# hangg7/soar

Measured on AMD Instinct MI355X. Metric: fwd+bwd frames/sec @100k Gaussians, 1080p; achieved HBM GB/s vs roofline, higher is better.
Workload: dtype f32

## Files before the change

include/soar_hip.h:

```cpp
#ifndef SOAR_HIP_H
#define SOAR_HIP_H

#include <stddef.h>
#include <stdint.h>

#ifdef __cplusplus
extern "C" {
#endif

#define SOAR_HIP_ABI_VERSION 8

typedef struct SoarRastParams {
    int32_t P;
    int32_t W, H;
    int32_t sh_degree;
    int32_t M;
    int32_t prefiltered;
    int32_t render_front;
    int32_t sort_descending;
    int32_t debug;
    int32_t cfg_surface;
    int32_t cfg_normalize_depth;
    int32_t cfg_perpix_depth;
    int32_t cfg_lrn_cam;
// ... 202 lines not shown
} SoarLossFinish;
int soar_frames_geometry_warp_backward_losses(int32_t n, const SoarFrameTail *frames, const float *xyz, const float *rot,
                                              const float *weights, const float *joint_mats, int32_t P, int32_t J, const float *scales,
                                              float *dL_dxyz, float *dL_drot, float *dL_dscales, float *dL_dcolors, float *dL_docc,
                                              const SoarLossFinish *finish, void *stream);

int soar_lbs_warp_forward_batch(const float *xyz, const float *rot, const float *weights, const float *joint_mats, int32_t n,
                                int32_t P, int32_t J, float *xyz_out, float *rot_out, void *stream);
int soar_lbs_warp_backward_sum(const float *xyz, const float *rot, const float *weights, const float *joint_mats, int32_t n,
                               int32_t P, int32_t J, const float *dL_dxyz_out, const float *dL_drot_out, float *dL_dxyz,
                               float *dL_drot, int32_t n_extra, const float *const *extra_src, float *const *extra_dst,
                               const int32_t *extra_width, void *stream);

int soar_dist2_knn3(const float *points, int32_t N, float *out, void *stream);

#define SOAR_FRAME_LOSS_SCRATCH_FLOATS (4 * 2048)
int soar_frame_loss(int32_t W, int32_t H, const float *color, const float *normal, const float *depth,
                    const float *opac, const float *target_color, const float *target_mask,
                    const float *target_normal, float w_color, float w_mask, float w_normal, float w_depth,
                    float *loss_out, float *scratch, float *dL_dcolor, float *dL_dnormal, float *dL_ddepth,
                    float *dL_dopac, const void *image_buffer, const float *background, int32_t normalize_depth, void *stream);

int soar_frame_loss_pooled(int32_t W, int32_t H, const float *color, const float *normal, const float *depth,
                           const float *opac, const float *target_pool, int32_t n_sets, const int32_t *set_index_dev,
                           float w_color, float w_mask, float w_normal, float w_depth, float *loss_out, float *scratch,
                           float *dL_dcolor, float *dL_dnormal, float *dL_ddepth, float *dL_dopac, const void *image_buffer,
                           const float *background, int32_t normalize_depth, void *stream);
int soar_frame_loss_partials(int32_t W, int32_t H, const float *color, const float *normal, const float *depth,
                             const float *opac, const float *target_color, const float *target_mask,
                             const float *target_normal, float w_color, float w_mask, float w_normal, float w_depth,
// ... 854 lines not shown
```

soar_amd/csrc/geom_bwd_point.h:

```cpp
#pragma once
#include "soar_common.h"
#include "soar_m3.h"

namespace soar {

namespace {

__constant__ float bSH_C0 = 0.28209479177387814f;
__constant__ float bSH_C1 = 0.4886025119029199f;
__constant__ float bSH_C2[5] = {1.0925484305920792f, -1.0925484305920792f, 0.31539156525252005f, -1.0925484305920792f,
                                0.5462742152960396f};
__constant__ float bSH_C3[7] = {-0.5900435899266435f, 2.890611442640554f, -0.4570457994644658f, 0.3731763325901154f,
                                -0.4570457994644658f, 1.445305721320277f, -0.5900435899266435f};

struct GeomBwdArgs {
    int P, D, M, W, H;
    int surface, lrn_cam;
    float tanfovx, tanfovy, h_x, h_y, scale_modifier;
    const float *means3D, *shs, *scales, *rotations, *cov3D;
    const int32_t *radii;
    const uint8_t *clamped;
    const float *view, *proj, *campos;
    const float *acc;
    float *dL_dmeans2D, *dL_dcolors, *dL_dopacity, *dL_dmeans3D, *dL_dcov3D, *dL_dsh, *dL_dscales, *dL_drots;
// ... 31 lines not shown
        acc[0] = r0.x; acc[1] = r0.y; acc[2] = r0.z; acc[3] = r0.w;
        acc[4] = r1.x; acc[5] = r1.y; acc[6] = r1.z; acc[7] = r1.w;
        acc[8] = r2.x; acc[9] = r2.y; acc[10] = r2.z; acc[11] = r2.w;
        acc[12] = r3.x; acc[13] = r3.y;
    }
#pragma unroll
    for (int k = 0; k < 3; k++) { g_mean[k] = 0.f; g_scale[k] = 0.f; }
#pragma unroll
    for (int k = 0; k < 6; k++) g_cov[k] = 0.f;
#pragma unroll
    for (int k = 0; k < 4; k++) g_rot[k] = 0.f;
    if (active) {
        const float *V = a.view, *PM = a.proj;
        const float mx = a.means3D[3 * idx], my = a.means3D[3 * idx + 1], mz = a.means3D[3 * idx + 2];

        const float *cov3D = a.cov3D + 6 * idx;
        const float dcon0 = acc[2], dcon1 = acc[3], dcon2 = acc[4];
        float t0 = V[0] * mx + V[4] * my + V[8] * mz + V[12];
        float t1 = V[1] * mx + V[5] * my + V[9] * mz + V[13];
        float t2 = V[2] * mx + V[6] * my + V[10] * mz + V[14];
        const float limx = 1.3f * a.tanfovx, limy = 1.3f * a.tanfovy;
        const float txtz = t0 / t2, tytz = t1 / t2;
        t0 = fminf(limx, fmaxf(-limx, txtz)) * t2;
        t1 = fminf(limy, fmaxf(-limy, tytz)) * t2;
        const float x_grad_mul = (txtz < -limx || txtz > limx) ? 0.f : 1.f;
        const float y_grad_mul = (tytz < -limy || tytz > limy) ? 0.f : 1.f;
        const float J0 = a.h_x / t2, J1 = -(a.h_x * t0) / (t2 * t2), J2 = a.h_y / t2, J3 = -(a.h_y * t1) / (t2 * t2);
        M3 Jm, Wm, Vrk;
        Jm.e[0][0] = J0; Jm.e[0][1] = 0.f; Jm.e[0][2] = J1;
        Jm.e[1][0] = 0.f; Jm.e[1][1] = J2; Jm.e[1][2] = J3;
        Jm.e[2][0] = 0.f; Jm.e[2][1] = 0.f; Jm.e[2][2] = 0.f;
// ... 123 lines not shown
                }
                ddir[0] += ddx * g; ddir[1] += ddy * g; ddir[2] += ddz * g;
            }
            const float sum2 = ox * ox + oy * oy + oz * oz;
            const float inv32 = 1.0f / sqrtf(sum2 * sum2 * sum2);
            const float gx_ = ((sum2 - ox * ox) * ddir[0] - oy * ox * ddir[1] - oz * ox * ddir[2]) * inv32;
            const float gy_ = (-ox * oy * ddir[0] + (sum2 - oy * oy) * ddir[1] - oz * oy * ddir[2]) * inv32;
            const float gz_ = (-ox * oz * ddir[0] - oy * oz * ddir[1] + (sum2 - oz * oz) * ddir[2]) * inv32;
            g_mean[0] += gx_; g_mean[1] += gy_; g_mean[2] += gz_;
            if ((CAM_SH && a.lrn_cam)) { cam_pos[0] -= gx_; cam_pos[1] -= gy_; cam_pos[2] -= gz_; }
        }

        if (a.scales) {
            const float4 q = reinterpret_cast<const float4 *>(a.rotations)[idx];
            const float r = q.x, x = q.y, y = q.z, z = q.w;
            M3 R, S;
            R.e[0][0] = 1.f - 2.f * (y * y + z * z); R.e[0][1] = 2.f * (x * y - r * z); R.e[0][2] = 2.f * (x * z + r * y);
            R.e[1][0] = 2.f * (x * y + r * z); R.e[1][1] = 1.f - 2.f * (x * x + z * z); R.e[1][2] = 2.f * (y * z - r * x);
            R.e[2][0] = 2.f * (x * z - r * y); R.e[2][1] = 2.f * (y * z + r * x); R.e[2][2] = 1.f - 2.f * (x * x + y * y);
            const float s0 = a.scale_modifier * a.scales[3 * idx], s1 = a.scale_modifier * a.scales[3 * idx + 1],
                        s2 = a.scale_modifier * a.scales[3 * idx + 2];
#pragma unroll
            for (int c = 0; c < 3; c++)
#pragma unroll
                for (int k = 0; k < 3; k++) S.e[c][k] = 0.f;
            S.e[0][0] = s0; S.e[1][1] = s1; S.e[2][2] = s2;
            M3 Mm = m3mul(S, R);
            M3 dSig;
            dSig.e[0][0] = g_cov[0]; dSig.e[0][1] = 0.5f * g_cov[1]; dSig.e[0][2] = 0.5f * g_cov[2];
            dSig.e[1][0] = 0.5f * g_cov[1]; dSig.e[1][1] = g_cov[3]; dSig.e[1][2] = 0.5f * g_cov[4];
            dSig.e[2][0] = 0.5f * g_cov[2]; dSig.e[2][1] = 0.5f * g_cov[4]; dSig.e[2][2] = g_cov[5];
#pragma unroll
            for (int c = 0; c < 3; c++)
#pragma unroll
// ... 29 lines not shown
        }
    }

}

inline void fill_geom_bwd_args(GeomBwdArgs &a, const SoarRastParams &prm, const float *means3D, const int32_t *radii, const float *shs,
                               const float *scales, const float *rotations, const float *cov3D_precomp, const GeomBuf &g, const float *acc)
{
    a.P = prm.P; a.D = prm.sh_degree; a.M = prm.M; a.W = prm.W; a.H = prm.H;
    a.surface = prm.cfg_surface; a.lrn_cam = prm.cfg_lrn_cam;
    a.tanfovx = prm.tanfovx; a.tanfovy = prm.tanfovy;
    a.h_y = prm.H / (2.0f * prm.tanfovy);
    a.h_x = prm.W / (2.0f * prm.tanfovx);
    a.scale_modifier = prm.scale_modifier;
    a.means3D = means3D; a.shs = shs; a.scales = scales; a.rotations = rotations;
    a.cov3D = cov3D_precomp ? cov3D_precomp : g.cov3D;
    a.radii = radii; a.clamped = g.clamped;
    a.view = prm.viewmatrix_dev; a.proj = prm.projmatrix_dev; a.campos = prm.campos_dev;
    a.acc = acc;
}

}

}
```

soar_amd/csrc/lbs.hip:

```cpp
#include "soar_common.h"
#include "loss_finish.h"
#include "geom_bwd_point.h"
#include "preprocess_point.h"
#include "soar_quat.h"

#pragma clang fp contract(on)

#ifndef SOAR_LBS_SKIP_UNUSED_JOINTS
#define SOAR_LBS_SKIP_UNUSED_JOINTS 1
#endif

namespace soar {

namespace {

constexpr int KNN_TILE = 1024;

__device__ __forceinline__ void quat_to_mat(const float q[4], float m[9])
{
    const float r = q[0], i = q[1], j = q[2], k = q[3];
    const float two_s = 2.0f / (r * r + i * i + j * j + k * k);
    m[0] = 1 - two_s * (j * j + k * k); m[1] = two_s * (i * j - k * r); m[2] = two_s * (i * k + j * r);
    m[3] = two_s * (i * j + k * r); m[4] = 1 - two_s * (i * i + k * k); m[5] = two_s * (j * k - i * r);
    m[6] = two_s * (i * k - j * r); m[7] = two_s * (j * k + i * r); m[8] = 1 - two_s * (i * i + j * j);
// ... 346 lines not shown
#pragma unroll
                for (int f = 0; f < WARP_NF; f++) v[c][f] = (c0 + c < w && f < n) ? src[(size_t)f * count + c0 + c] : 0.f;
#pragma unroll
            for (int c = 0; c < 4; c++) {
                if (c0 + c >= w) break;
                float s = v[c][0];
#pragma unroll
                for (int f = 1; f < WARP_NF; f++) s = f < n ? s + v[c][f] : s;
                for (int f = WARP_NF; f < n; f++) s += src[(size_t)f * count + c0 + c];
                dst[c0 + c] = s;
            }
        }
    }
}

__global__ void __launch_bounds__(WARP_THREADS) warp_preprocess_frames_kernel(WarpArgs a, int n, Batch<PreArgs> fr)
{
    extern __shared__ float wtile[];
    const int tid = threadIdx.x, k = __builtin_amdgcn_readfirstlane(tid / WAVE), lane = tid % WAVE;
    const int p0 = blockIdx.x * WAVE, p_raw = p0 + lane;
    stage_weight_rows(a, wtile, tid, p0);
    const int f = blockIdx.y * WARP_NF + k;
    if (f >= n) return;
    const bool in_range = p_raw < a.P;
    const int p = in_range ? p_raw : a.P - 1;
    float M[12], pos[3];
    float4 quat;
    blend_frame_matrix(wtile + (p - p0) * a.J, a.joint_mats + (size_t)f * a.mats_stride, a.J, M);
    forward_point_vals(a, p, M, pos, quat);
    float *xyz_out = a.xyz_out + (size_t)f * a.xyz_stride, *rot_out = a.rot_out + (size_t)f * a.rot_stride;
    xyz_out[3 * p] = pos[0]; xyz_out[3 * p + 1] = pos[1]; xyz_out[3 * p + 2] = pos[2];
    reinterpret_cast<float4 *>(rot_out)[p] = quat;
    const PreArgs &g = fr.v[f];
    PrePoint o;
    preprocess_point(g, p, in_range, pos[0], pos[1], pos[2], true, quat, o);
    preprocess_store(g, p, in_range, blockIdx.x, o);
    if (!g.prefiltered && blockIdx.x == 0 && lane == 0) g.header[H_PREFILTER_VIOLATIONS] = 0u;
}

constexpr int TAIL_C = 14;
struct TailOut {
    float *dL_dmeans2D[MAX_BATCH];
    float *dL_dscales, *dL_dcolors, *dL_docc;
};
struct TailLosses {
    int n, first_block;
    int per_wave;
    SoarLossFinish v[MAX_BATCH];
};
#ifndef SOAR_TAIL_WPE
#define SOAR_TAIL_WPE 4
// ... 47 lines not shown
#pragma unroll
                for (int kk = 0; kk < WARP_NF; kk++) acc[h] += red[kk * TAIL_C * WAVE + o];
        }
    }
#pragma unroll
    for (int h = 0; h < PER; h++) {
        const int o = tid + h * WARP_THREADS, c = o / WAVE, q = p0 + o % WAVE;
        if (o < TAIL_C * WAVE && q < a.P) {
            if (c < 3) a.g_xyz[3 * q + c] = acc[h];
            else if (c < 7) a.g_rot[4 * q + c - 3] = acc[h];
            else if (c < 10) out.dL_dscales[3 * q + c - 7] = acc[h];
            else if (c < 13) out.dL_dcolors[3 * q + c - 10] = acc[h];
            else if (out.dL_docc) out.dL_docc[q] = acc[h];
        }
    }
}

__global__ void __launch_bounds__(256) dist2_knn3_kernel(const float *__restrict__ pts, int N, float *__restrict__ out)
{
    __shared__ float tile[KNN_TILE * 3];
    const int tid = threadIdx.x;
    const int p = blockIdx.x * 256 + tid;
    const bool valid = p < N;
    float x = 0.f, y = 0.f, z = 0.f;
    if (valid) { x = pts[3 * p]; y = pts[3 * p + 1]; z = pts[3 * p + 2]; }
    float b0 = 3.402823466e+38f, b1 = b0, b2 = b0;
    for (int base = 0; base < N; base += KNN_TILE) {
        const int n = min(KNN_TILE, N - base);
        __syncthreads();
        for (int t = tid; t < n * 3; t += 256) tile[t] = pts[(size_t)base * 3 + t];
// ... 153 lines not shown
    a.P = P; a.J = J; a.xyz = xyz; a.rot = rot; a.weights = weights; a.joint_mats = joint_mats;
    a.xyz_out = xyz_out; a.rot_out = rot_out;
    a.mats_stride = (size_t)J * 16; a.xyz_stride = (size_t)P * 3; a.rot_stride = (size_t)P * 4;
    Batch<PreArgs> fr{};
    for (int f = 0; f < n; f++) {
        const SoarFrameHead &t = frames[f];
        if (!t.prm || !t.geom_buffer || !t.radii) { set_error("%s: frame %d: a pointer is NULL", who, f); return 1; }
        if (t.prm->P != P || t.prm->M != 0 || t.prm->prefiltered != 0) {
            set_error("%s: frame %d: needs P = %d Gaussians with explicit colours (M = 0), not prefiltered", who, f, P);
            return 1;
        }
        GeomBuf g;
        carve_geom(t.geom_buffer, P, 0, &g);
        fill_pre_args(fr.v[f], *t.prm, xyz_out + (size_t)f * a.xyz_stride, nullptr, colors, opacities, scales, rot_out + (size_t)f * a.rot_stride,
                      nullptr, g, t.radii);
    }
    const size_t lds = sizeof(float) * WAVE * (size_t)J;
    StageTimer timer(ST_LBS_WARP_FWD, stream);
    hipLaunchKernelGGL(warp_preprocess_frames_kernel, dim3((P + WAVE - 1) / WAVE, (n + WARP_NF - 1) / WARP_NF), dim3(WARP_THREADS), lds, stream,
                       a, (int)n, fr);
    SOAR_LAUNCH_OK("frames_warp_preprocess", stream, 0);
    return 0;
}

int soar_frames_geometry_warp_backward(int32_t n, const SoarFrameTail *frames, const float *xyz, const float *rot, const float *weights,
                                       const float *joint_mats, int32_t P, int32_t J, const float *scales, float *dL_dxyz, float *dL_drot,
                                       float *dL_dscales, float *dL_dcolors, float *dL_docc, void *stream_)
{
    return soar_frames_geometry_warp_backward_losses(n, frames, xyz, rot, weights, joint_mats, P, J, scales, dL_dxyz, dL_drot, dL_dscales,
                                                     dL_dcolors, dL_docc, nullptr, stream_);
}

// ... 61 lines not shown
            if (!l.sums4 || !l.loss_out || l.blocks < 1 || l.blocks > SOAR_FRAME_LOSS_SCRATCH_FLOATS / 4 || l.n < 1) {
                set_error("%s: frame %d: finish[] is not what %s left", who, f,
                          per_wave ? "soar_rast_backward_plan_loss" : "soar_frame_loss_partials");
                return 1;
            }
            losses.v[f] = l;
        }
    }
    const size_t lds = sizeof(float) * (WAVE * (size_t)J + WARP_NF * TAIL_C * WAVE);
    StageTimer timer(ST_LBS_WARP_BWD, stream);
    hipLaunchKernelGGL(geom_warp_backward_frames_kernel, dim3(blocks + losses.n), dim3(WARP_THREADS), lds, stream, a, (int)n, fr, out, losses);
    SOAR_LAUNCH_OK("frames_geometry_warp_backward", stream, 0);
    return 0;
}

int soar_dist2_knn3(const float *points, int32_t N, float *out, void *stream_)
{
    hipStream_t stream = static_cast<hipStream_t>(stream_);
    if (N < 0) { set_error("soar_dist2_knn3: N < 0"); return 1; }
    if (N == 0) return 0;
    if (!points || !out) { set_error("soar_dist2_knn3: NULL pointer"); return 1; }
    StageTimer timer(ST_DIST2, stream);
    hipLaunchKernelGGL(dist2_knn3_kernel, dim3((N + 255) / 256), dim3(256), 0, stream, points, N, out);
    SOAR_LAUNCH_OK("dist2_knn3", stream, 0);
    return 0;
}

}
```

soar_amd/csrc/preprocess_point.h:

```cpp
#pragma once
#include "soar_common.h"
#include "soar_m3.h"

namespace soar {

namespace {

__device__ __forceinline__ float pix_from_ndc(float v, int S, float prcp)
{
#pragma clang fp contract(off)
    return (float)(((v + 1.0) * S - 1.0) * 0.5 + S * (prcp - 0.5));
}

__device__ __forceinline__ float unit3(float *v)
{
#pragma clang fp contract(off)
    float mod = fmaxf(sqrtf(v[0] * v[0] + v[1] * v[1] + v[2] * v[2]), (float)0.00000001);
    v[0] /= mod;
    v[1] /= mod;
    v[2] /= mod;
    return mod;
}

__constant__ float kSH_C0 = 0.28209479177387814f;
// ... 59 lines not shown
    uint8_t *clamped;
    float *front_out;
    uint2 *rect_out;
    uint32_t *depth_key_out;
    uint32_t *blk_stats;
    int32_t *radii;
    uint32_t *header;
};

struct PrePoint {
    GaussRec rec;
    uint2 rect;
    uint32_t depth_key, tiles, key_bits;
    int radius;
    bool alive, faces_camera, prefilter_violation;
};

__device__ __forceinline__ void preprocess_point(const PreArgs &a, const int idx, const bool in_range, const float px3, const float py3,
                                                 const float pz3, const bool has_rot, const float4 q, PrePoint &o)
{
#pragma clang fp contract(off)
    int out_radius = 0;
    uint32_t out_tiles = 0;
    uint2 out_rect = make_uint2(0u, 0u);
    GaussRec rec;
    rec.q0 = make_float4(0.f, 0.f, 0.f, 0.f);
    rec.q1 = rec.q0;
    rec.q2 = rec.q0;
    rec.q3 = rec.q0;

// ... 14 lines not shown
    bool alive = true;
    {
        float x0 = a.bbox[1], y0 = a.bbox[0], x1 = a.bbox[3], y1 = a.bbox[2];
        float w = x1 - x0, h = y1 - y0;
        float expand = (float)0.2;
        if (vz < 0 || pix_x < x0 - w * expand || pix_x >= x1 + w * expand || pix_y < y0 - h * expand ||
            pix_y >= y1 + h * expand)
            alive = false;
    }
    bool prefilter_violation = a.prefiltered && in_range && !alive;

    M3 R;
    if (alive) {
        float r = 1.f, x = 0.f, y = 0.f, z = 0.f;
        if (has_rot) { r = q.x; x = q.y; y = q.z; z = q.w; }
        R.e[0][0] = 1.f - 2.f * (y * y + z * z); R.e[0][1] = 2.f * (x * y - r * z); R.e[0][2] = 2.f * (x * z + r * y);
        R.e[1][0] = 2.f * (x * y + r * z); R.e[1][1] = 1.f - 2.f * (x * x + z * z); R.e[1][2] = 2.f * (y * z - r * x);
        R.e[2][0] = 2.f * (x * z - r * y); R.e[2][1] = 2.f * (y * z + r * x); R.e[2][2] = 1.f - 2.f * (x * x + y * y);
    }

    float nview[3] = {0.f, 0.f, 0.f};
    float plane_a = 0.f, plane_b = 0.f;
    bool faces_camera = true;
    if (alive && a.surface) {
        float ax0[3], ax1[3];
#pragma unroll
        for (int k = 0; k < 3; k++) {
            nview[k] = V[k] * R.e[0][2] + V[4 + k] * R.e[1][2] + V[8 + k] * R.e[2][2];
            ax0[k] = V[k] * R.e[0][0] + V[4 + k] * R.e[1][0] + V[8 + k] * R.e[2][0];
            ax1[k] = V[k] * R.e[0][1] + V[4 + k] * R.e[1][1] + V[8 + k] * R.e[2][1];
        }
        float dot = vx * nview[0] + vy * nview[1] + vz * nview[2];
        bool front = !((double)dot > -0.01);
// ... 28 lines not shown
                float J[4];
                J[0] = xu0[0] * ax0[0] + xu0[1] * ax0[1] + xu0[2] * ax0[2];
                J[1] = xu1[0] * ax0[0] + xu1[1] * ax0[1] + xu1[2] * ax0[2];
                J[2] = xu0[0] * ax1[0] + xu0[1] * ax1[1] + xu0[2] * ax1[2];
                J[3] = xu1[0] * ax1[0] + xu1[1] * ax1[1] + xu1[2] * ax1[2];
                float sc = Svp / S_fix;
                J[0] /= sc; J[1] /= sc; J[2] /= sc; J[3] /= sc;
                plane_a = ax0[2] * J[0] + ax1[2] * J[2];
                plane_b = ax0[2] * J[1] + ax1[2] * J[3];
            }
        }
    }

    float cv[6] = {0, 0, 0, 0, 0, 0};
    float conic[3] = {0, 0, 0};
    if (alive) {
        if (a.cov3D_precomp) {
#pragma unroll
            for (int k = 0; k < 6; k++) cv[k] = a.cov3D_precomp[6 * idx + k];
        } else {
            const float mod = a.scale_modifier;
            M3 S;
#pragma unroll
            for (int c = 0; c < 3; c++)
#pragma unroll
                for (int k = 0; k < 3; k++) S.e[c][k] = (c == k) ? 1.f : 0.f;
            S.e[0][0] = mod * a.scales[3 * idx + 0];
            S.e[1][1] = mod * a.scales[3 * idx + 1];
            S.e[2][2] = ((mod * (a.surface ? 1.0f : 0.0f)) != 0.0f) ? 0.f : a.scales[3 * idx + 2];
            M3 Mm = m3mul(S, R);
            M3 Sg = m3mul(m3t(Mm), Mm);
            cv[0] = Sg.e[0][0]; cv[1] = Sg.e[0][1]; cv[2] = Sg.e[0][2];
            cv[3] = Sg.e[1][1]; cv[4] = Sg.e[1][2]; cv[5] = Sg.e[2][2];
#pragma unroll
            for (int k = 0; k < 6; k++) a.cov3D[6 * idx + k] = cv[k];
        }

        float t0 = vx, t1 = vy, t2 = vz;
        const float limx = 1.3f * a.tanfovx, limy = 1.3f * a.tanfovy;
        const float txtz = t0 / t2, tytz = t1 / t2;
        t0 = fminf(limx, fmaxf(-limx, txtz)) * t2;
        t1 = fminf(limy, fmaxf(-limy, tytz)) * t2;
        M3 Jm, Wm, Vrk;
        Jm.e[0][0] = a.focal_x / t2; Jm.e[0][1] = 0.0f; Jm.e[0][2] = -(a.focal_x * t0) / (t2 * t2);
        Jm.e[1][0] = 0.0f; Jm.e[1][1] = a.focal_y / t2; Jm.e[1][2] = -(a.focal_y * t1) / (t2 * t2);
        Jm.e[2][0] = 0.f; Jm.e[2][1] = 0.f; Jm.e[2][2] = 0.f;
        Wm.e[0][0] = V[0]; Wm.e[0][1] = V[4]; Wm.e[0][2] = V[8];
        Wm.e[1][0] = V[1]; Wm.e[1][1] = V[5]; Wm.e[1][2] = V[9];
        Wm.e[2][0] = V[2]; Wm.e[2][1] = V[6]; Wm.e[2][2] = V[10];
        Vrk.e[0][0] = cv[0]; Vrk.e[0][1] = cv[1]; Vrk.e[0][2] = cv[2];
// ... 34 lines not shown
        if (a.colors) {
            rgb[0] = a.colors[3 * idx]; rgb[1] = a.colors[3 * idx + 1]; rgb[2] = a.colors[3 * idx + 2];
        } else {
            unsigned f = sh_to_rgb(idx, a.D, a.M, a.means3D, a.campos, a.shs, rgb);
            a.clamped[3 * idx + 0] = f & 1u;
            a.clamped[3 * idx + 1] = (f >> 1) & 1u;
            a.clamped[3 * idx + 2] = (f >> 2) & 1u;
        }
        rec.q0 = make_float4(pix_x, pix_y, conic[0], conic[1]);
        rec.q1 = make_float4(conic[2], a.opacities[idx], vz, plane_a);
        rec.q2 = make_float4(plane_b, rgb[0], rgb[1], rgb[2]);
        rec.q3 = make_float4(nview[0], nview[1], nview[2], splat_cull_threshold(a.opacities[idx]));
    }
    o.rec = rec; o.rect = out_rect; o.depth_key = alive ? __float_as_uint(vz) : 0xFFFFFFFFu; o.key_bits = __float_as_uint(vz);
    o.tiles = out_tiles; o.radius = out_radius; o.alive = alive; o.faces_camera = faces_camera; o.prefilter_violation = prefilter_violation;
}

__device__ __forceinline__ void preprocess_store(const PreArgs &a, const int idx, const bool in_range, const int stats_row, const PrePoint &o)
{
    a.rec[idx] = o.rec;
    a.rect_out[idx] = o.rect;
    a.depth_key_out[idx] = o.depth_key;
    {
        const bool vis = o.alive && in_range;
        const uint32_t key = o.key_bits;
        uint32_t v[BLK_STATS] = {vis ? key : 0u, vis ? ~key : 0u, vis ? (o.rect.x >> 16) : 0u, vis ? (o.rect.y >> 16) : 0u,
                                 vis ? ~(o.rect.x & 0xFFFFu) : 0u, vis ? ~(o.rect.y & 0xFFFFu) : 0u};
#pragma unroll
        for (int k = 0; k < BLK_STATS; k++) {
#pragma unroll
            for (int off = 32; off > 0; off >>= 1) v[k] = max(v[k], (uint32_t)__shfl_xor((int)v[k], off));
        }
        if (stats_row >= 0 && (threadIdx.x & 63) < BLK_STATS) {
            const int k = threadIdx.x & 63;
            a.blk_stats[stats_row * BLK_STATS + k] = k == 0 ? v[0] : k == 1 ? v[1] : k == 2 ? v[2] : k == 3 ? v[3] : k == 4 ? v[4] : v[5];
        }
    }
    a.front_out[idx] = o.faces_camera ? 1.f : 0.f;
    a.radii[idx] = o.radius;
    a.tiles_touched[idx] = o.tiles;
    if (a.prefiltered) {
        const unsigned long long bad = __ballot(o.prefilter_violation);
        if (bad != 0ull && (threadIdx.x & 63) == 0) atomicAdd(a.header + H_PREFILTER_VIOLATIONS, (uint32_t)__builtin_popcountll(bad));
    }
}

inline void fill_pre_args(PreArgs &a, const SoarRastParams &prm, const float *means3D, const float *shs, const float *colors_precomp,
                          const float *opacities, const float *scales, const float *rotations, const float *cov3D_precomp, GeomBuf &g,
                          int32_t *radii)
{
    a.P = prm.P; a.D = prm.sh_degree; a.M = prm.M; a.W = prm.W; a.H = prm.H;
    a.gx = (prm.W + TILE - 1) / TILE; a.gy = (prm.H + TILE - 1) / TILE;
    a.prefiltered = prm.prefiltered; a.render_front = prm.render_front;
    a.surface = prm.cfg_surface; a.pix_depth = prm.cfg_perpix_depth;
    a.tanfovx = prm.tanfovx; a.tanfovy = prm.tanfovy;
    a.focal_y = prm.H / (2.0f * prm.tanfovy);
    a.focal_x = prm.W / (2.0f * prm.tanfovx);
    a.scale_modifier = prm.scale_modifier;
    a.means3D = means3D; a.shs = shs; a.colors = colors_precomp; a.opacities = opacities;
// ... 11 lines not shown
```

soar_amd/csrc/soar_m3.h:

```cpp
#pragma once
#include "soar_common.h"

namespace soar {

namespace {

struct M3 {
    float e[3][3];
};
__device__ __forceinline__ M3 m3mul(const M3 &a, const M3 &b)
{
#pragma clang fp contract(off)
    M3 r;
#pragma unroll
    for (int c = 0; c < 3; c++)
#pragma unroll
        for (int k = 0; k < 3; k++) r.e[c][k] = a.e[0][k] * b.e[c][0] + a.e[1][k] * b.e[c][1] + a.e[2][k] * b.e[c][2];
    return r;
}
__device__ __forceinline__ M3 m3t(const M3 &a)
{
#pragma clang fp contract(off)
    M3 r;
#pragma unroll
    for (int c = 0; c < 3; c++)
#pragma unroll
        for (int k = 0; k < 3; k++) r.e[c][k] = a.e[k][c];
    return r;
}

}

}
```

soar_amd/hip_lib.py:

```python
from __future__ import annotations

import ctypes as C
import os
from typing import Optional

import torch

_HERE = os.path.dirname(os.path.abspath(__file__))
LIB_PATH = os.environ.get("SOAR_HIP_LIB") or os.path.join(_HERE, "_lib", "libsoar_hip.so")
if os.environ.get("SOAR_HIP_LIB"):
    import sys as _sys
    print(f"[soar_amd] SOAR_HIP_LIB is set: loading {LIB_PATH} instead of the in-tree build (development A/B runs only)", file=_sys.stderr)

FRAME_LOSS_SCRATCH_FLOATS = 4 * 2048
ABI_VERSION = 8
c_f32p = C.c_void_p
_vp = C.c_void_p


class SoarRastParams(C.Structure):
    _fields_ = [
        ("P", C.c_int32), ("W", C.c_int32), ("H", C.c_int32), ("sh_degree", C.c_int32), ("M", C.c_int32),
        ("prefiltered", C.c_int32), ("render_front", C.c_int32), ("sort_descending", C.c_int32), ("debug", C.c_int32),
        ("cfg_surface", C.c_int32), ("cfg_normalize_depth", C.c_int32), ("cfg_perpix_depth", C.c_int32),
# ... 369 lines not shown
    "soar_lbs_knn_query_ordered": (C.c_int, [_vp, C.c_int32, _vp, C.c_int32, _vp, C.c_int32, C.c_int32, _vp, C.c_int32, _vp, _vp,
                                             _vp, C.c_size_t, _vp]),
    "soar_lbs_knn_state_bytes": (C.c_int, [C.c_int32, C.POINTER(C.c_size_t)]),
    "soar_lbs_knn_query_state": (C.c_int, [_vp, C.c_int32, _vp, C.c_int32, _vp, C.c_int32, _vp, C.c_int32, _vp, _vp, _vp, C.c_size_t, _vp]),
    "soar_lbs_knn_refresh": (C.c_int, [_vp, C.c_int32, C.c_int32, _vp, C.c_int32, _vp, _vp, _vp, _vp, _vp]),
    "soar_lbs_warp_forward": (C.c_int, [_vp] * 6 + [C.c_int32, C.c_int32] + [_vp] * 4),
    "soar_lbs_warp_backward": (C.c_int, [_vp] * 5 + [C.c_int32, C.c_int32] + [_vp] * 5),
    "soar_lbs_warp_forward_batch": (C.c_int, [_vp] * 4 + [C.c_int32] * 3 + [_vp] * 3),
    "soar_lbs_warp_backward_sum": (C.c_int, [_vp] * 4 + [C.c_int32] * 3 + [_vp] * 4 + [C.c_int32, _vp, _vp, _vp, _vp]),
    "soar_frames_warp_preprocess": (C.c_int, [C.c_int32, _vp] + [_vp] * 4 + [C.c_int32, C.c_int32] + [_vp] * 6),
    "soar_rast_backward_rows": (C.c_int, [_vp] * 22),
    "soar_frames_geometry_warp_backward": (C.c_int, [C.c_int32, _vp] + [_vp] * 4 + [C.c_int32, C.c_int32] + [_vp] * 7),
    "soar_frames_geometry_warp_backward_losses": (C.c_int, [C.c_int32, _vp] + [_vp] * 4 + [C.c_int32, C.c_int32] + [_vp] * 8),
    "soar_frames_geometry_warp_backward_wave_losses": (C.c_int, [C.c_int32, _vp] + [_vp] * 4 + [C.c_int32, C.c_int32] + [_vp] * 8),
    "soar_dist2_knn3": (C.c_int, [_vp, C.c_int32, _vp, _vp]),
    "soar_depth2normal": (C.c_int, [C.c_int32, C.c_int32, _vp, _vp, C.c_float, C.c_float, C.c_float, C.c_float, _vp, _vp]),
    "soar_depth2normal_backward": (C.c_int, [C.c_int32, C.c_int32, _vp, _vp, C.c_float, C.c_float, C.c_float, C.c_float, _vp, _vp,
                                             _vp]),
    "soar_normal2curv": (C.c_int, [C.c_int32, C.c_int32, _vp, _vp, _vp, _vp]),
    "soar_normal2curv_backward": (C.c_int, [C.c_int32, C.c_int32, _vp, _vp, _vp, _vp, _vp]),
    "soar_view_finish": (C.c_int, [C.c_int32, C.c_int32, _vp, _vp, _vp, _vp, C.c_float, C.c_float, _vp, _vp, _vp, _vp]),
    "soar_view_finish_backward": (C.c_int, [C.c_int32, C.c_int32, _vp, _vp, _vp, _vp, C.c_float, C.c_float, _vp, _vp, _vp, _vp,
                                            _vp, _vp]),
    "soar_ssim_scratch_floats": (C.c_int, [C.c_int32, C.c_int32, C.c_int32, C.POINTER(C.c_size_t)]),
    "soar_ssim": (C.c_int, [C.c_int32, C.c_int32, C.c_int32, _vp, _vp, _vp, _vp, _vp, _vp]),
    "soar_ssim_rendered": (C.c_int, [C.c_int32, C.c_int32, C.c_int32, _vp, _vp, _vp, _vp, _vp, _vp, _vp]),
    "soar_densify_stats": (C.c_int, [C.c_int32, _vp, _vp, C.c_int32, _vp, _vp, _vp, _vp, _vp, _vp]),
    "soar_densify_plan_bytes": (C.c_int, [C.c_int32, C.POINTER(C.c_size_t)]),
    "soar_densify_plan": (C.c_int, [C.c_int32, _vp, _vp, _vp, C.c_int32, C.c_int32, C.c_float, C.c_float, C.c_float, C.c_float,
                                    C.c_float, _vp, C.POINTER(C.c_int64), _vp]),
# ... 263 lines not shown
```

soar_amd/step_plan.py:

```python
from __future__ import annotations

import ctypes as C
import os
from typing import Dict, List, Optional, Sequence

import torch

from . import hip_lib
from .hip_lib import check, ptr
from .rasterizer import _Ctx


class FrameStepPlan:
    def __init__(self, seq, n_frames: int, targets: Dict[str, torch.Tensor], bg: torch.Tensor, capacity: int, flat,
                 loss_weights: Sequence[float] = (1.0, 1.0, 0.1, 0.01), use_graphs: bool = True, batched: Optional[bool] = None,
                 loss: str = "synthetic", lambdas: Optional[Dict[str, float]] = None):
        if loss not in ("synthetic", "avatar"):
            raise ValueError(f"loss must be 'synthetic' or 'avatar', got {loss!r}")
        self.loss_kind = loss
        if loss == "avatar" and (use_graphs or not torch.is_tensor(targets)):
            raise ValueError("loss='avatar' needs a resident target pool and use_graphs=False")
        L = hip_lib.lib()
        self.L, self.seq, self.flat, self.n = L, seq, flat, int(n_frames)
        dev = seq.device
# ... 50 lines not shown
            self._tail_frames = (hip_lib.SoarFrameTail * self.n)()
            for i, v in enumerate(self.views):
                t = self._tail_frames[i]
                t.prm = C.addressof(self.ctx.params)
                t.means3D, t.rotations, t.radii = v["xyz_p"].data_ptr(), v["rot_p"].data_ptr(), v["radii"].data_ptr()
                t.geom_buffer, t.workspace, t.dL_dmeans2D = v["geom"].data_ptr(), v["work"].data_ptr(), v["g_means2D"].data_ptr()
        env = os.environ.get("SOAR_PLAN_BWD_REGION")
        self.bwd_region = int(env) if env in ("1", "2") else (2 if W * H >= (1 << 20) else 1)
        self.fused_head = os.environ.get("SOAR_PLAN_FUSED_HEAD", "1") != "0" and self.n <= 8
        if self.fused_head:
            self.ctx.params.debug |= 16
            self._head_frames = (hip_lib.SoarFrameHead * self.n)()
            for i, v in enumerate(self.views):
                h = self._head_frames[i]
                h.prm, h.geom_buffer, h.radii = C.addressof(self.ctx.params), v["geom"].data_ptr(), v["radii"].data_ptr()
        self.g_xyz = torch.empty((self.n, P, 3), **f)
        self.g_rot = torch.empty((self.n, P, 4), **f)
        self.g_scales = torch.empty((self.n, P, 3), **f)
        self.g_colors = torch.empty((self.n, P, 3), **f)
        self.losses = torch.empty((self.n,), **f)
        from . import lbs as _lbs
        self.knn = _lbs.KnnFollower(seq.knn_grid, P)
        for name in ("opacity", "occ"):
            if name in flat.views:
                flat.views[name].zero_()
        if loss == "avatar":
            self._setup_avatar(lambdas)
        self.steps = 0
        self.STAMP_CAP = 8192
        self.stamps = torch.zeros((1 + 2 * self.STAMP_CAP,), dtype=torch.int64, device=dev) if os.environ.get("SOAR_PLAN_TIMESTAMPS") in ("1", "2") else None
# ... 465 lines not shown
```

Measured before the change: 5807.

## Recompute cov3D in backward instead of storing it; stage fused-head stores via LDS

When both the fused head and fused tail are active, a new debug flag (on by default) stops the warp/preprocess kernel from writing per-point 3D covariances to memory. The geometry backward kernel then recomputes them from scales and rotations, trading a 6-float write plus read per point per frame for extra arithmetic. The fused head kernel also stages its rec, xyz and cov stores through LDS with a swizzle so the global writes are coalesced, which enlarges the LDS allocation. A standalone cov3D kernel and shared quaternion and covariance helpers are added.

```diff
diff --git a/include/soar_hip.h b/include/soar_hip.h
--- a/include/soar_hip.h
+++ b/include/soar_hip.h
@@ -240,6 +240,8 @@
 
 int soar_dist2_knn3(const float *points, int32_t N, float *out, void *stream);
 
+int soar_lbs_cov3d(const float *scales, const float *rotations, int32_t P, float scale_modifier, int32_t surface, float *cov3D, void *stream);
+
 #define SOAR_FRAME_LOSS_SCRATCH_FLOATS (4 * 2048)
 int soar_frame_loss(int32_t W, int32_t H, const float *color, const float *normal, const float *depth,
                     const float *opac, const float *target_color, const float *target_mask,
diff --git a/soar_amd/csrc/geom_bwd_point.h b/soar_amd/csrc/geom_bwd_point.h
--- a/soar_amd/csrc/geom_bwd_point.h
+++ b/soar_amd/csrc/geom_bwd_point.h
@@ -69,7 +69,15 @@
         const float *V = a.view, *PM = a.proj;
         const float mx = a.means3D[3 * idx], my = a.means3D[3 * idx + 1], mz = a.means3D[3 * idx + 2];
 
-        const float *cov3D = a.cov3D + 6 * idx;
+        float cov3D[6];
+        if (a.cov3D == nullptr) {
+            const float4 q = reinterpret_cast<const float4 *>(a.rotations)[idx];
+            cov3d_from_scales_rot(a.scale_modifier, a.surface, a.scales[3 * idx], a.scales[3 * idx + 1], a.scales[3 * idx + 2],
+                                  m3quat(q.x, q.y, q.z, q.w), cov3D);
+        } else {
+#pragma unroll
+            for (int k = 0; k < 6; k++) cov3D[k] = a.cov3D[6 * idx + k];
+        }
         const float dcon0 = acc[2], dcon1 = acc[3], dcon2 = acc[4];
         float t0 = V[0] * mx + V[4] * my + V[8] * mz + V[12];
         float t1 = V[1] * mx + V[5] * my + V[9] * mz + V[13];
@@ -223,10 +231,8 @@
         if (a.scales) {
             const float4 q = reinterpret_cast<const float4 *>(a.rotations)[idx];
             const float r = q.x, x = q.y, y = q.z, z = q.w;
-            M3 R, S;
-            R.e[0][0] = 1.f - 2.f * (y * y + z * z); R.e[0][1] = 2.f * (x * y - r * z); R.e[0][2] = 2.f * (x * z + r * y);
-            R.e[1][0] = 2.f * (x * y + r * z); R.e[1][1] = 1.f - 2.f * (x * x + z * z); R.e[1][2] = 2.f * (y * z - r * x);
-            R.e[2][0] = 2.f * (x * z - r * y); R.e[2][1] = 2.f * (y * z + r * x); R.e[2][2] = 1.f - 2.f * (x * x + y * y);
+            M3 S;
+            const M3 R = m3quat(r, x, y, z);
             const float s0 = a.scale_modifier * a.scales[3 * idx], s1 = a.scale_modifier * a.scales[3 * idx + 1],
                         s2 = a.scale_modifier * a.scales[3 * idx + 2];
 #pragma unroll
@@ -286,7 +292,7 @@
     a.h_x = prm.W / (2.0f * prm.tanfovx);
     a.scale_modifier = prm.scale_modifier;
     a.means3D = means3D; a.shs = shs; a.scales = scales; a.rotations = rotations;
-    a.cov3D = cov3D_precomp ? cov3D_precomp : g.cov3D;
+    a.cov3D = cov3D_precomp ? cov3D_precomp : ((prm.debug & 32) && scales && rotations) ? nullptr : g.cov3D;
     a.radii = radii; a.clamped = g.clamped;
     a.view = prm.viewmatrix_dev; a.proj = prm.projmatrix_dev; a.campos = prm.campos_dev;
     a.acc = acc;
diff --git a/soar_amd/csrc/lbs.hip b/soar_amd/csrc/lbs.hip
--- a/soar_amd/csrc/lbs.hip
+++ b/soar_amd/csrc/lbs.hip
@@ -384,27 +384,76 @@
     }
 }
 
+constexpr int HEAD_STAGE = 16 * WAVE;
+__device__ __forceinline__ void wave_lds_handover()
+{
+    __builtin_amdgcn_fence(__ATOMIC_RELEASE, "wavefront", "local");
+    __builtin_amdgcn_wave_barrier();
+    __builtin_amdgcn_fence(__ATOMIC_ACQUIRE, "wavefront", "local");
+}
 __global__ void __launch_bounds__(WARP_THREADS) warp_preprocess_frames_kernel(WarpArgs a, int n, Batch<PreArgs> fr)
 {
-    extern __shared__ float wtile[];
+    extern __shared__ __attribute__((aligned(16))) float wtile[];
     const int tid = threadIdx.x, k = __builtin_amdgcn_readfirstlane(tid / WAVE), lane = tid % WAVE;
     const int p0 = blockIdx.x * WAVE, p_raw = p0 + lane;
     stage_weight_rows(a, wtile, tid, p0);
     const int f = blockIdx.y * WARP_NF + k;
-    if (f >= n) return;
+    const bool live = f < n;
     const bool in_range = p_raw < a.P;
     const int p = in_range ? p_raw : a.P - 1;
-    float M[12], pos[3];
-    float4 quat;
-    blend_frame_matrix(wtile + (p - p0) * a.J, a.joint_mats + (size_t)f * a.mats_stride, a.J, M);
-    forward_point_vals(a, p, M, pos, quat);
-    float *xyz_out = a.xyz_out + (size_t)f * a.xyz_stride, *rot_out = a.rot_out + (size_t)f * a.rot_stride;
-    xyz_out[3 * p] = pos[0]; xyz_out[3 * p + 1] = pos[1]; xyz_out[3 * p + 2] = pos[2];
+    float pos[3] = {0.f, 0.f, 0.f};
+    float4 quat = make_float4(0.f, 0.f, 0.f, 0.f);
+    PrePoint o;
+    if (live) {
+        float M[12];
+        blend_frame_matrix(wtile + (p - p0) * a.J, a.joint_mats + (size_t)f * a.mats_stride, a.J, M);
+        forward_point_vals(a, p, M, pos, quat);
+        preprocess_point(fr.v[f], p, in_range, pos[0], pos[1], pos[2], true, quat, o);
+    }
+    __syncthreads();
+    if (!live) return;
+    const PreArgs &g = fr.v[f];
+    const int cnt = min(WAVE, a.P - p0);
+    float *st = wtile + k * HEAD_STAGE;
+    float4 *st4 = reinterpret_cast<float4 *>(st);
+    {
+        const int sw = (lane >> 2) & 3;
+        st4[4 * lane + (0 ^ sw)] = o.rec.q0; st4[4 * lane + (1 ^ sw)] = o.rec.q1;
+        st4[4 * lane + (2 ^ sw)] = o.rec.q2; st4[4 * lane + (3 ^ sw)] = o.rec.q3;
+        wave_lds_handover();
+        float4 *rec_out = reinterpret_cast<float4 *>(g.rec + p0);
+#pragma unroll
+        for (int c = 0; c < 4; c++) {
+            const int m = c * WAVE + lane;
+            if (m < 4 * cnt) rec_out[m] = st4[(m & ~3) | ((m & 3) ^ ((m >> 4) & 3))];
+        }
+        wave_lds_handover();
+    }
+    float *st_cov = st + 3 * WAVE;
+#pragma unroll
+    for (int c = 0; c < 3; c++) st[3 * lane + c] = pos[c];
+    if (g.cov3D) {
+#pragma unroll
+        for (int c = 0; c < 6; c++) st_cov[6 * lane + c] = o.cov[c];
+    }
+    const unsigned long long made = __ballot(o.cov_made);
+    wave_lds_handover();
+    float *xyz_out = a.xyz_out + (size_t)f * a.xyz_stride + (size_t)3 * p0, *rot_out = a.rot_out + (size_t)f * a.rot_stride;
+#pragma unroll
+    for (int c = 0; c < 3; c++) {
+        const int m = c * WAVE + lane;
+        if (m < 3 * cnt) xyz_out[m] = st[m];
+    }
+    if (g.cov3D) {
+        float *cov_out = g.cov3D + (size_t)6 * p0;
+#pragma unroll
+        for (int c = 0; c < 6; c++) {
+            const int m = c * WAVE + lane;
+            if (m < 6 * cnt && ((made >> (m / 6)) & 1ull)) cov_out[m] = st_cov[m];
+        }
+    }
     reinterpret_cast<float4 *>(rot_out)[p] = quat;
-    const PreArgs &g = fr.v[f];
-    PrePoint o;
-    preprocess_point(g, p, in_range, pos[0], pos[1], pos[2], true, quat, o);
-    preprocess_store(g, p, in_range, blockIdx.x, o);
+    preprocess_store_rest(g, p, in_range, blockIdx.x, o);
     if (!g.prefiltered && blockIdx.x == 0 && lane == 0) g.header[H_PREFILTER_VIOLATIONS] = 0u;
 }
 
@@ -482,6 +531,18 @@
             else if (out.dL_docc) out.dL_docc[q] = acc[h];
         }
     }
+}
+
+__global__ void __launch_bounds__(256) cov3d_kernel(const float *__restrict__ scales, const float *__restrict__ rotations, int P, float mod, int surface,
+                                                    float *__restrict__ cov3D)
+{
+    const int p = blockIdx.x * 256 + threadIdx.x;
+    if (p >= P) return;
+    const float4 q = reinterpret_cast<const float4 *>(rotations)[p];
+    float cv[6];
+    cov3d_from_scales_rot(mod, surface, scales[3 * p], scales[3 * p + 1], scales[3 * p + 2], m3quat(q.x, q.y, q.z, q.w), cv);
+#pragma unroll
+    for (int k = 0; k < 6; k++) cov3D[6 * p + k] = cv[k];
 }
 
 __global__ void __launch_bounds__(256) dist2_knn3_kernel(const float *__restrict__ pts, int N, float *__restrict__ out)
@@ -665,8 +726,10 @@
         carve_geom(t.geom_buffer, P, 0, &g);
         fill_pre_args(fr.v[f], *t.prm, xyz_out + (size_t)f * a.xyz_stride, nullptr, colors, opacities, scales, rot_out + (size_t)f * a.rot_stride,
                       nullptr, g, t.radii);
-    }
-    const size_t lds = sizeof(float) * WAVE * (size_t)J;
+        if (t.prm->debug & 32) fr.v[f].cov3D = nullptr;
+    }
+    static_assert(WARP_MAXJ * WAVE <= WARP_NF * HEAD_STAGE, "the staging area of the stores covers the weight tile");
+    const size_t lds = sizeof(float) * WARP_NF * HEAD_STAGE;
     StageTimer timer(ST_LBS_WARP_FWD, stream);
     hipLaunchKernelGGL(warp_preprocess_frames_kernel, dim3((P + WAVE - 1) / WAVE, (n + WARP_NF - 1) / WARP_NF), dim3(WARP_THREADS), lds, stream,
                        a, (int)n, fr);
@@ -758,6 +821,17 @@
     return 0;
 }
 
+int soar_lbs_cov3d(const float *scales, const float *rotations, int32_t P, float scale_modifier, int32_t surface, float *cov3D, void *stream_)
+{
+    hipStream_t stream = static_cast<hipStream_t>(stream_);
+    if (P < 0) { set_error("soar_lbs_cov3d: P < 0"); return 1; }
+    if (P == 0) return 0;
+    if (!scales || !rotations || !cov3D) { set_error("soar_lbs_cov3d: NULL pointer"); return 1; }
+    hipLaunchKernelGGL(cov3d_kernel, dim3((P + 255) / 256), dim3(256), 0, stream, scales, rotations, P, scale_modifier, surface, cov3D);
+    SOAR_LAUNCH_OK("lbs_cov3d", stream, 0);
+    return 0;
+}
+
 int soar_dist2_knn3(const float *points, int32_t N, float *out, void *stream_)
 {
     hipStream_t stream = static_cast<hipStream_t>(stream_);
diff --git a/soar_amd/csrc/preprocess_point.h b/soar_amd/csrc/preprocess_point.h
--- a/soar_amd/csrc/preprocess_point.h
+++ b/soar_amd/csrc/preprocess_point.h
@@ -97,6 +97,8 @@
     uint32_t depth_key, tiles, key_bits;
     int radius;
     bool alive, faces_camera, prefilter_violation;
+    float cov[6];
+    bool cov_made;
 };
 
 __device__ __forceinline__ void preprocess_point(const PreArgs &a, const int idx, const bool in_range, const float px3, const float py3,
@@ -141,9 +143,7 @@
     if (alive) {
         float r = 1.f, x = 0.f, y = 0.f, z = 0.f;
         if (has_rot) { r = q.x; x = q.y; y = q.z; z = q.w; }
-        R.e[0][0] = 1.f - 2.f * (y * y + z * z); R.e[0][1] = 2.f * (x * y - r * z); R.e[0][2] = 2.f * (x * z + r * y);
-        R.e[1][0] = 2.f * (x * y + r * z); R.e[1][1] = 1.f - 2.f * (x * x + z * z); R.e[1][2] = 2.f * (y * z - r * x);
-        R.e[2][0] = 2.f * (x * z - r * y); R.e[2][1] = 2.f * (y * z + r * x); R.e[2][2] = 1.f - 2.f * (x * x + y * y);
+        R = m3quat(r, x, y, z);
     }
 
     float nview[3] = {0.f, 0.f, 0.f};
@@ -202,26 +202,14 @@
 
     float cv[6] = {0, 0, 0, 0, 0, 0};
     float conic[3] = {0, 0, 0};
+    bool cov_made = false;
     if (alive) {
         if (a.cov3D_precomp) {
 #pragma unroll
             for (int k = 0; k < 6; k++) cv[k] = a.cov3D_precomp[6 * idx + k];
         } else {
-            const float mod = a.scale_modifier;
-            M3 S;
-#pragma unroll
-            for (int c = 0; c < 3; c++)
-#pragma unroll
-                for (int k = 0; k < 3; k++) S.e[c][k] = (c == k) ? 1.f : 0.f;
-            S.e[0][0] = mod * a.scales[3 * idx + 0];
-            S.e[1][1] = mod * a.scales[3 * idx + 1];
-            S.e[2][2] = ((mod * (a.surface ? 1.0f : 0.0f)) != 0.0f) ? 0.f : a.scales[3 * idx + 2];
-            M3 Mm = m3mul(S, R);
-            M3 Sg = m3mul(m3t(Mm), Mm);
-            cv[0] = Sg.e[0][0]; cv[1] = Sg.e[0][1]; cv[2] = Sg.e[0][2];
-            cv[3] = Sg.e[1][1]; cv[4] = Sg.e[1][2]; cv[5] = Sg.e[2][2];
-#pragma unroll
-            for (int k = 0; k < 6; k++) a.cov3D[6 * idx + k] = cv[k];
+            cov3d_from_scales_rot(a.scale_modifier, a.surface, a.scales[3 * idx + 0], a.scales[3 * idx + 1], a.scales[3 * idx + 2], R, cv);
+            cov_made = true;
         }
 
         float t0 = vx, t1 = vy, t2 = vz;
@@ -286,11 +274,13 @@
     }
     o.rec = rec; o.rect = out_rect; o.depth_key = alive ? __float_as_uint(vz) : 0xFFFFFFFFu; o.key_bits = __float_as_uint(vz);
     o.tiles = out_tiles; o.radius = out_radius; o.alive = alive; o.faces_camera = faces_camera; o.prefilter_violation = prefilter_violation;
-}
-
-__device__ __forceinline__ void preprocess_store(const PreArgs &a, const int idx, const bool in_range, const int stats_row, const PrePoint &o)
-{
-    a.rec[idx] = o.rec;
+#pragma unroll
+    for (int k = 0; k < 6; k++) o.cov[k] = cv[k];
+    o.cov_made = cov_made;
+}
+
+__device__ __forceinline__ void preprocess_store_rest(const PreArgs &a, const int idx, const bool in_range, const int stats_row, const PrePoint &o)
+{
     a.rect_out[idx] = o.rect;
     a.depth_key_out[idx] = o.depth_key;
     {
@@ -315,6 +305,15 @@
         const unsigned long long bad = __ballot(o.prefilter_violation);
         if (bad != 0ull && (threadIdx.x & 63) == 0) atomicAdd(a.header + H_PREFILTER_VIOLATIONS, (uint32_t)__builtin_popcountll(bad));
     }
+}
+__device__ __forceinline__ void preprocess_store(const PreArgs &a, const int idx, const bool in_range, const int stats_row, const PrePoint &o)
+{
+    a.rec[idx] = o.rec;
+    if (o.cov_made) {
+#pragma unroll
+        for (int k = 0; k < 6; k++) a.cov3D[6 * idx + k] = o.cov[k];
+    }
+    preprocess_store_rest(a, idx, in_range, stats_row, o);
 }
 
 inline void fill_pre_args(PreArgs &a, const SoarRastParams &prm, const float *means3D, const float *shs, const float *colors_precomp,
diff --git a/soar_amd/csrc/soar_m3.h b/soar_amd/csrc/soar_m3.h
--- a/soar_amd/csrc/soar_m3.h
+++ b/soar_amd/csrc/soar_m3.h
@@ -29,6 +29,33 @@
     return r;
 }
 
+__device__ __forceinline__ M3 m3quat(float r, float x, float y, float z)
+{
+#pragma clang fp contract(off)
+    M3 R;
+    R.e[0][0] = 1.f - 2.f * (y * y + z * z); R.e[0][1] = 2.f * (x * y - r * z); R.e[0][2] = 2.f * (x * z + r * y);
+    R.e[1][0] = 2.f * (x * y + r * z); R.e[1][1] = 1.f - 2.f * (x * x + z * z); R.e[1][2] = 2.f * (y * z - r * x);
+    R.e[2][0] = 2.f * (x * z - r * y); R.e[2][1] = 2.f * (y * z + r * x); R.e[2][2] = 1.f - 2.f * (x * x + y * y);
+    return R;
+}
+
+__device__ __forceinline__ void cov3d_from_scales_rot(float mod, int surface, float sx, float sy, float sz, const M3 &R, float cv[6])
+{
+#pragma clang fp contract(off)
+    M3 S;
+#pragma unroll
+    for (int c = 0; c < 3; c++)
+#pragma unroll
+        for (int k = 0; k < 3; k++) S.e[c][k] = (c == k) ? 1.f : 0.f;
+    S.e[0][0] = mod * sx;
+    S.e[1][1] = mod * sy;
+    S.e[2][2] = ((mod * (surface ? 1.0f : 0.0f)) != 0.0f) ? 0.f : sz;
+    M3 Mm = m3mul(S, R);
+    M3 Sg = m3mul(m3t(Mm), Mm);
+    cv[0] = Sg.e[0][0]; cv[1] = Sg.e[0][1]; cv[2] = Sg.e[0][2];
+    cv[3] = Sg.e[1][1]; cv[4] = Sg.e[1][2]; cv[5] = Sg.e[2][2];
 }
 
 }
+
+}
diff --git a/soar_amd/hip_lib.py b/soar_amd/hip_lib.py
--- a/soar_amd/hip_lib.py
+++ b/soar_amd/hip_lib.py
@@ -407,6 +407,7 @@
     "soar_frames_geometry_warp_backward_losses": (C.c_int, [C.c_int32, _vp] + [_vp] * 4 + [C.c_int32, C.c_int32] + [_vp] * 8),
     "soar_frames_geometry_warp_backward_wave_losses": (C.c_int, [C.c_int32, _vp] + [_vp] * 4 + [C.c_int32, C.c_int32] + [_vp] * 8),
     "soar_dist2_knn3": (C.c_int, [_vp, C.c_int32, _vp, _vp]),
+    "soar_lbs_cov3d": (C.c_int, [_vp, _vp, C.c_int32, C.c_float, C.c_int32, _vp, _vp]),
     "soar_depth2normal": (C.c_int, [C.c_int32, C.c_int32, _vp, _vp, C.c_float, C.c_float, C.c_float, C.c_float, _vp, _vp]),
     "soar_depth2normal_backward": (C.c_int, [C.c_int32, C.c_int32, _vp, _vp, C.c_float, C.c_float, C.c_float, C.c_float, _vp, _vp,
                                              _vp]),
diff --git a/soar_amd/step_plan.py b/soar_amd/step_plan.py
--- a/soar_amd/step_plan.py
+++ b/soar_amd/step_plan.py
@@ -88,6 +88,9 @@
             for i, v in enumerate(self.views):
                 h = self._head_frames[i]
                 h.prm, h.geom_buffer, h.radii = C.addressof(self.ctx.params), v["geom"].data_ptr(), v["radii"].data_ptr()
+        self.cov3D_in_registers = self.fused_head and self.fused_tail and os.environ.get("SOAR_PLAN_COV3D_IN_REGISTERS", "1") != "0"
+        if self.cov3D_in_registers:
+            self.ctx.params.debug |= 32
         self.g_xyz = torch.empty((self.n, P, 3), **f)
         self.g_rot = torch.empty((self.n, P, 4), **f)
         self.g_scales = torch.empty((self.n, P, 3), **f)
```

After: 5836 (median of 6 runs). Within noise of the previous version (+0.5%).
